# nyx-space/nyx

Hardware: AMD Instinct MI355X
Metric: propagated trajectories/sec (10k-ensemble, 1-day RK89) (higher is better)
Workload: dtype f64

## Files before the change

### nyx_amd/csrc/pk_integrator_ool.h

```cpp
#ifndef INTEG_OOL
#define INTEG_OOL ((NYX_EMIT & (NYX_EMIT_PLAIN16 | NYX_EMIT_PLAIN16_P2 | NYX_EMIT_PLAIN16_FAN)) ? 1 : 0)
#endif
#if INTEG_OOL
#define IX_HOT 1
#define IX_SPEC_NOW 2
#define IX_COOP 4
#define IX_PROF 8
#define IX_SHARED 16
#define IXR_ANSWER 0x10000
#define IXR_FALLBACK 0x20000
DEVFN char *lds_from_u32(uint32_t a) { return (char *)(__attribute__((address_space(3))) char *)(uintptr_t)a; }
DEVFN LdsPtr ix_rows(const double *arr, int lane) {
    uint32_t a = (uint32_t)(uintptr_t)(LdsCPtr)arr + (uint32_t)lane * 8u;
    asm volatile("" : "+v"(a));
    return (LdsPtr)(uintptr_t)a;
}
DEVFN void ix_stamp(LdsFlagPtr ctl, int k) {
    const int64_t t = (int64_t)__builtin_readcyclecounter();
    ctl[8 + 2 * k] = (int)(uint32_t)t; ctl[9 + 2 * k] = (int)(uint32_t)(t >> 32);
}
#define IX_PROLOGUE                                                                                                        \
    CfgPtr cfg = (CfgPtr)uniform_u64(cfg_u);                                                                               \
    const LdsMap L = carve_lds(lds_from_u32(__builtin_amdgcn_readfirstlane(lds_v)), 0, false, cfg->rec_in_lds ? cfg->rec_doubles : 0, cfg->ed_reuse, false); \
    double *const kbuf = L.kbuf;                                                                                           \
    double *const tabl = L.tabl;                                                                                           \
    constexpr int KB_STR = DEV_LANES;                                                                                      \
    const int kb_li = lane;                                                                                                \
    const int i = __builtin_amdgcn_readfirstlane(i_v);                                                                     \
    const int flags = __builtin_amdgcn_readfirstlane(flags_v);                                                             \
    const int stages = cfg->stages;

static __device__ __attribute__((noinline)) int integ_front(uint32_t lds_v, uint64_t cfg_u, int i_v, int flags_v, int lane, double h,
                                                           double v3, double v4, double v5, double p0, double p1, double p2,
                                                           uint64_t cbox_u, uint64_t posted_u, uint32_t seq_nx_v, int keep_k0) {
    IX_PROLOGUE
    const bool has_grav = cfg->has_grav != 0;
    const bool need_almanac = has_grav || cfg->has_drag != 0 || cfg->has_tides != 0 || cfg->n_slots > 0;
    const bool spec = cfg->spec != 0;
    int st = NYX_HIP_OK;
    double vel[3] = {v3, v4, v5};
    if (flags & IX_HOT) {
        double *const ysb = (i & 1) ? L.ys2 : L.ys;
        if (i == 0) {
#pragma unroll
            for (int e = 0; e < 3; ++e) vel[e] = CS_Y(3 + e);
        } else {
            const double a_last = A_ROW(i, i - 1);
            const double w[3] = {v3, v4, v5};
#pragma unroll
            for (int e = 0; e < 3; ++e) {
                const double wi = w[e] + a_last * KB(i - 1, 3 + e);
                vel[e] = CS_Y(3 + e) + h * wi;
            }
        }
#pragma unroll
        for (int e = 0; e < 3; ++e) ysb[(3 + e) * DEV_LANES + lane] = vel[e];
        if (cfg->has_drag) {
            __builtin_amdgcn_fence(__ATOMIC_RELEASE, "workgroup");
            if (lane == 0) LCTL[4] = i + 1;
        }
        if (need_almanac && !(i == 0 && keep_k0)) {
            const int n_alm = cfg->n_alm;
            for (int a = 0; a < n_alm; ++a) {
                const int es = L.edst[(2 * a + (i & 1)) * DEV_LANES + lane];
                if (es) st = es;
            }
        }
// ... 15 lines not shown
        }
        double *const ysn = ((i + 1) & 1) ? L.ys2 : L.ys;
        double *const inbn = ((i + 1) & 1) ? L.inb2 : L.inb;
#pragma unroll
        for (int e = 0; e < 3; ++e) ysn[e * DEV_LANES + lane] = nx_pos[e];
        if (has_grav) {
            if (need_almanac) {
                int spin = 0;
                while (LCTL[2] != i + 1 && ++spin < 4000000) __builtin_amdgcn_s_sleep(4);
                if (spin >= 4000000) st = NYX_HIP_ERR_NAN;
                __builtin_amdgcn_fence(__ATOMIC_ACQUIRE, "workgroup");
            }
            const double *const edn = L.ed + ((i + 1) & 1) * ED_FIELDS * DEV_LANES;
            double m_nx[9];
#pragma unroll
            for (int q = 0; q < 9; ++q) m_nx[q] = edn[q * DEV_LANES + lane];
            const double rb0 = m_nx[0] * nx_pos[0] + m_nx[1] * nx_pos[1] + m_nx[2] * nx_pos[2];
            const double rb1 = m_nx[3] * nx_pos[0] + m_nx[4] * nx_pos[1] + m_nx[5] * nx_pos[2];
            const double rb2 = m_nx[6] * nx_pos[0] + m_nx[7] * nx_pos[1] + m_nx[8] * nx_pos[2];
            const double r_ = norm3(rb0, rb1, rb2);
            const double inv_r = 1.0 / r_;
            const double nx_s = rb0 * inv_r, nx_t = rb1 * inv_r, nx_u = rb2 * inv_r;
            const double rho = cfg->g_re * inv_r;
            const double nx_kfac = (cfg->g_mu * inv_r) * cfg->g_inv_re;
            inbn[0 * DEV_LANES + lane] = rho * nx_s;
            inbn[1 * DEV_LANES + lane] = rho * nx_t;
            inbn[2 * DEV_LANES + lane] = rho * nx_u;
            inbn[3 * DEV_LANES + lane] = rho;
            inbn[4 * DEV_LANES + lane] = r_ * cfg->g_inv_re;
            double *const sx = ((i + 1) & 1) ? L.ixs : L.part;
            sx[0 * DEV_LANES + lane] = nx_s; sx[1 * DEV_LANES + lane] = nx_t; sx[2 * DEV_LANES + lane] = nx_u; sx[3 * DEV_LANES + lane] = nx_kfac;
        }
        if (lane == 0) L.ctl[1] = (flags & IX_COOP) ? 1 : 0;
        if ((flags & IX_COOP) && has_grav) {
            CoopBox *const cbox = (CoopBox *)uniform_u64(cbox_u);
            uint32_t *const posted = (uint32_t *)uniform_u64(posted_u);
            const uint32_t seq_nx = (uint32_t)__builtin_amdgcn_readfirstlane((int)seq_nx_v);
            if (flags & IX_PROF) ix_stamp(LCTL, 1);
            coop_post_inl(cbox, posted, lane, seq_nx, (LdsCPtr)inbn, COOP_PARTS_HERE);
            if (flags & IX_PROF) ix_stamp(LCTL, 2);
        }
    }
    return st;
}

struct IxBack {
    double px, py, pz, pw;
    int ret;
};
#define IXR_NEED_FB 0x40000
DEVFN void ix_assemble(CfgPtr cfg, const LdsMap &L, int i, int lane, double (&acc)[3], double px, double py, double pz, double pw,
                       const double (&m_cur)[9], double s_, double t_, double u_, double kfac, int skip_k) {
    const LdsPtr pertc = ix_rows((i & 1) ? L.pert2 : L.pert, lane);
    const LdsPtr ysb = ix_rows((i & 1) ? L.ys2 : L.ys, lane);
    const LdsPtr kb = ix_rows(L.kbuf + i * 6 * DEV_LANES, lane);
    if (cfg->has_grav) {
        px *= kfac; py *= kfac; pz *= kfac; pw *= kfac;
        const double al0 = px + pw * s_, al1 = py + pw * t_, al2 = pz + pw * u_;
        acc[0] += m_cur[0] * al0 + m_cur[3] * al1 + m_cur[6] * al2;
        acc[1] += m_cur[1] * al0 + m_cur[4] * al1 + m_cur[7] * al2;
        acc[2] += m_cur[2] * al0 + m_cur[5] * al1 + m_cur[8] * al2;
    }
    if (cfg->has_srp) {
        acc[0] += pertc[3 * DEV_LANES]; acc[1] += pertc[4 * DEV_LANES]; acc[2] += pertc[5 * DEV_LANES];
    }
    if (cfg->has_drag) {
        acc[0] += pertc[6 * DEV_LANES]; acc[1] += pertc[7 * DEV_LANES]; acc[2] += pertc[8 * DEV_LANES];
    }
    if (!skip_k) {
        kb[0 * DEV_LANES] = ysb[3 * DEV_LANES]; kb[1 * DEV_LANES] = ysb[4 * DEV_LANES]; kb[2 * DEV_LANES] = ysb[5 * DEV_LANES];
        kb[3 * DEV_LANES] = acc[0]; kb[4 * DEV_LANES] = acc[1]; kb[5 * DEV_LANES] = acc[2];
    }
}
static __device__ __attribute__((noinline)) IxBack integ_back(uint32_t lds_v, uint64_t cfg_u, int i_v, int flags_v, int lane, double a0, double a1,
                                                             double a2, double px, double py, double pz, double pw, uint32_t seq_cur_v, int fold_val_v,
// ... 210 lines not shown
```

### nyx_amd/csrc/pk_state_lds.h

```cpp

#define NIN 5
#define DBG_SKIP_SERIAL 0x100
#define DBG_SKIP_HARMONICS 0x200
#define KB(stage, comp) kbuf[((stage)*6 + (comp)) * KB_STR + kb_li]

#define CS_FIELDS 21
static __device__ __attribute__((noinline)) bool event_step(const nyx_hip_event_t *ev, double mu, int64_t epoch_ns, double *prev, int32_t *count,
                                                            double y0, double y1, double y2, double y3, double y4, double y5) {
    const double y[6] = {y0, y1, y2, y3, y4, y5};
    const double y_next = ev_eval(*ev, mu, epoch_ns, y);
    int n = *count;
    if (ev_crossing(ev->scalar, *prev, y_next)) n += 1;
    *prev = y_next;
    *count = n;
    return n >= ev->trigger;
}

struct ColdState {
    int64_t epoch, stop, step_size, prev_step, det_step, n_acc, n_rej, n_evals;
    double y[9];
    double h, det_error;
    int det_attempts, attempts, status;
    bool done, fresh, is_final, fixed, prev_kind, backprop, massless;
};
// ... 108 lines not shown
               2 * ED_FIELDS * DEV_LANES + 2 * DEV_LANES + CS_FIELDS * DEV_LANES + (size_t)(quad ? DEV_MAX_WAVES * QSLOT : DEV_MAX_WAVES * 4 * DEV_LANES) + DEV_MAX_ALM * DEV_LANES +
               DEV_LANES + 8 + (size_t)rec_doubles;
    d += quad ? (size_t)(10 + 15 + 6 + QPRE_ROWS + 6 + 10 + 15) * DEV_LANES : (stm ? (size_t)(20 + 27 + 12) * DEV_LANES : (size_t)(NIN + 9 + 6 + NIN + 9 + 4) * DEV_LANES);
    (void)n_waves;
    if (reuse_fields > 0) d += (size_t)reuse_fields * DEV_LANES + 2 * DEV_LANES + DEV_LANES / 2;
    return d * sizeof(double) + 64;
}

DEVFN void begin_attempt_fn(const LdsMap &L, int lane, ColdState &c) {
    if (!c.done && c.fresh) {
        if ((!c.backprop && c.epoch + c.step_size > c.stop) || (c.backprop && c.epoch + c.step_size <= c.stop)) {
            if (c.stop == c.epoch) {
                c.done = true;
            } else {
                c.prev_step = c.step_size;
                c.prev_kind = c.fixed;
                c.step_size = c.stop - c.epoch;
                c.fixed = true;
                c.is_final = true;
            }
        }
        c.attempts = 1;
        c.h = ns_to_seconds(c.step_size);
        c.fresh = false;
    }
    if (!c.done && c.massless) { c.status = NYX_HIP_ERR_MASSLESS; c.done = true; }
    L.step[lane] = __longlong_as_double(c.epoch);
    L.step[DEV_LANES + lane] = c.h;
    if (!__any(!c.done)) {
        if (lane == 0) L.ctl[0] = 1;
    }
}

#define PROF_T0() const int64_t pt0_ = prof_on ? (int64_t)__builtin_readcyclecounter() : 0
#define PROF_ADD(slot) if (prof_on) prof_acc[slot] += (int64_t)__builtin_readcyclecounter() - pt0_
#define A_ROW(i, j) tabl[(i)*DEV_MAX_STAGES + (j)]
#define B_COEF(i) tabl[DEV_MAX_STAGES * DEV_MAX_STAGES + (i)]
#define BD_COEF(i) tabl[DEV_MAX_STAGES * DEV_MAX_STAGES + DEV_MAX_STAGES + (i)]
#define C_COEF(i) tabl[DEV_MAX_STAGES * DEV_MAX_STAGES + 2 * DEV_MAX_STAGES + (i)]

static __device__ __attribute__((noinline)) bool stm_update_textbook(double *phi, double h, const double *hist, int64_t stride, int64_t gid, double *kb,
                                                                  const double *tabl, int stages_v, int lane) {
    const int stages = __builtin_amdgcn_readfirstlane(stages_v);
    bool nan = false;
    for (int col = 0; col < 9; ++col) {
        double p[6];
#pragma unroll
        for (int e = 0; e < 6; ++e) p[e] = phi[e + 9 * col];
        const double gam = phi[6 + 9 * col];
        for (int i = 0; i < stages; ++i) {
            double wi[6] = {0.0, 0.0, 0.0, 0.0, 0.0, 0.0};
            for (int j = 0; j < i; ++j) {
                const double a_ij = A_ROW(i, j);
#pragma unroll
                for (int e = 0; e < 6; ++e) wi[e] += a_ij * kb[(j * 6 + e) * DEV_LANES + lane];
            }
            double ps[6];
#pragma unroll
            for (int e = 0; e < 6; ++e) ps[e] = p[e] + h * wi[e];
            double g[12];
#pragma unroll
            for (int q = 0; q < 12; ++q) g[q] = hist[(int64_t)(i * 12 + q) * stride + gid];
#pragma unroll
            for (int a = 0; a < 3; ++a) {
                double s = g[3 * a + 0] * ps[0];
                s += g[3 * a + 1] * ps[1];
// ... 25 lines not shown
```

### nyx_amd/csrc/propagate_kernel.hip

```cpp

#include <hip/hip_runtime.h>

#include <mutex>

#include "../../include/nyx_hip.h"
#include "devcfg.h"
#include "hifitime_dev.h"
#include "event_dev.h"
#include "predict_args.h"

#ifndef NYX_EMIT
#define NYX_EMIT 1
#endif
#define NYX_EMIT_PLAIN16 1
#define NYX_EMIT_PLAIN8 2
#define NYX_EMIT_STM 4
#define NYX_EMIT_STMQ16 8
#define NYX_EMIT_STMQ8 16
#define NYX_EMIT_PLAIN16_P2 32
#define NYX_EMIT_PLAIN8N 64
#define NYX_EMIT_PLAIN16_FAN 128
#ifndef NYX_PROF
#define NYX_PROF 0
#endif
#define NYX_HOST_TU ((NYX_EMIT & NYX_EMIT_PLAIN16) && !NYX_PROF)
#ifdef NYX_COOP_TWO_PARTS
#define COOP_PARTS_HERE 2
#else
#define COOP_PARTS_HERE 1
#endif

#define CAS __attribute__((address_space(4)))
typedef const CAS DevCfg *CfgPtr;
typedef const CAS HarmEntry *HarmPtr;
typedef const CAS ColHdr *ColPtr;

#define DEVFN static __device__ __forceinline__
typedef const __attribute__((address_space(3))) double *LdsCPtr;
typedef volatile __attribute__((address_space(3))) int *LdsFlagPtr;
#define LCTL ((LdsFlagPtr)L.ctl)

DEVFN double norm3(double x, double y, double z) { return sqrt(x * x + y * y + z * z); }
DEVFN double cube(double x) { return x * (x * x); }
DEVFN double clamp02(double x) { return x < 0.0 ? 0.0 : (x > 2.0 ? 2.0 : x); }

#include "pk_epoch_data.h"
#include "pk_force_models.h"
#include "pk_harmonics.h"
#include "pk_cooperative.h"
#include "pk_error_stm.h"
#include "pk_state_lds.h"
#include "pk_integrator_ool.h"
#include "pk_segment_update.h"
template <bool INTEG, bool ALMANAC, bool PERT, bool STM, bool QUAD = false, bool PIPE = false>
DEVFN void role_loop(const DevBatch &bt, CfgPtr cfg, const DevCfg *cfg_g, HarmPtr htab, ColPtr cols,
                     const double *__restrict__ records, const LdsMap &L, const int lane, const int wave, const int nw) {
    double *const kbuf = L.kbuf;
    double *const tabl = L.tabl;
    const int stages = cfg->stages;
    asm volatile("s_nop 13\n\ts_nop %0" ::"n"((INTEG ? 1 : 0) | (ALMANAC ? 2 : 0) | (PERT ? 4 : 0) | (PIPE ? 8 : 0)) : "memory");
#ifdef NYX_ASSUME_SMALL
    const bool has_grav = false, has_drag = false, has_tides = false, has_grav2 = false;
// ... 62 lines not shown
        }
        if (bt.traj_cap > 0 && wr) {
            bt.t_epoch[gid] = c.epoch;
#pragma unroll
            for (int e = 0; e < 6; ++e) bt.t_state[e][gid] = c.y[e];
            bt.t_len[gid] = (duration == 0 || c.done) ? 1 : 1;
        }
        if (STM && valid && bt.o_stm != bt.stm) {
            for (int q = ql; q < 81; q += (QUAD ? 4 : 1)) bt.o_stm[gid * 81 + q] = bt.stm[gid * 81 + q];
        }
    }
    if (PERT) {
        p_cr = clamp02(bt.cr ? bt.cr[idx] : 0.0);
        p_area = bt.asrp ? bt.asrp[idx] : 0.0;
        p_cd = bt.cd ? bt.cd[idx] : 0.0;
        p_darea = bt.adrag ? bt.adrag[idx] : 0.0;
        p_mass = (bt.mdry ? bt.mdry[idx] : 0.0) + (bt.mprop ? bt.mprop[idx] : 0.0) + (bt.mextra ? bt.mextra[idx] : 0.0);
    }
    __syncthreads();
    CoopBox *const cbox = bt.coop_box + blockIdx.x;
    const int coop_widx = bt.coop_sets > 0 ? ((int)blockIdx.x % bt.coop_sets) * COOP_SET + (int)blockIdx.x / bt.coop_sets : 0;
#define coop_two (COOP_PARTS_HERE == 2)
#ifdef NYX_COOP_FAN
#define COOP_FB_PARTS ((bt.coop_parts & 0xf) << 8)
#else
#define COOP_FB_PARTS (coop_two ? 0x100 : 0)
#endif
    bool coop_on = !STM && LCTL[1] != 0;
    const bool coop_started = coop_on;
    uint32_t coop_seq = 0;
    bool coop_drop = false;
    static_assert(!PIPE || ((!STM || QUAD) && !(INTEG && (ALMANAC || PERT))), "the pipelined stage loop needs the integrator in a wave of its own");
    constexpr bool pipe = PIPE;
    RotBase rot_base;
    rot_base.ep = INT64_MIN;
#pragma unroll
    for (int q = 0; q < 3; ++q) { rot_base.sn[q] = 0.0; rot_base.cs[q] = 1.0; }
    const int reuse_nf = (!STM && ALMANAC && !INTEG && need_almanac && cfg->n_alm == 1) ? cfg->ed_reuse : 0;
    if (reuse_nf > 0) { L.ed0_ep[lane] = INT64_MIN; L.spec_ep[lane] = INT64_MIN; }
    const bool spec = pipe && !STM && cfg->spec != 0;
    const bool offl = PIPE && !STM && !INTEG_OOL && cfg->offload != 0;
    const bool qoff = STM && QUAD && cfg->qpre_off != 0;
#if INTEG_OOL
    constexpr bool ool = PIPE && !STM;
    const uint32_t lds_base = (uint32_t)(uintptr_t)(LdsPtr)L.kbuf;
#define IX_STAMP(k) (int64_t)(((uint64_t)(uint32_t)LCTL[9 + 2 * (k)] << 32) | (uint64_t)(uint32_t)LCTL[8 + 2 * (k)])
#else
    constexpr bool ool = false;
#endif
    bool spec_now = false;
    bool keep_k0 = false;
    int att = 0;
    double nx_pos[3] = {0.0, 0.0, 0.0}, nx_s = 0.0, nx_t = 0.0, nx_u = 0.0, nx_kfac = 0.0;
    double m_cur[9], m_nx[9];
#pragma unroll
    for (int q = 0; q < 9; ++q) { m_cur[q] = 0.0; m_nx[q] = 0.0; }
    uint32_t seq_cur = 0, seq_nx = 0;
    unsigned long long dbg_answers = 0, dbg_fallbacks = 0, dbg_fb_seq = 0;
    int64_t pl_tc = 0, pl_chain = 0, pl_wait = 0, pl_n = 0, pl_post = 0;
#if NYX_SEG_PROF
    int64_t sg[16] = {0, 0, 0, 0, 0, 0, 0, 0, 0, 0, 0, 0, 0, 0, 0, 0}, sg_t = 0;
#define SEG(k) if (INTEG && prof_on) { const int64_t n_ = (int64_t)__builtin_readcyclecounter(); sg[k] += n_ - sg_t; sg_t = n_; }
    int64_t sb[8] = {0, 0, 0, 0, 0, 0, 0, 0}, sb_t = 0;
#define SBD(k) if (INTEG && STM && prof_on) { const int64_t n_ = (int64_t)__builtin_readcyclecounter(); if (sb_t) sb[k] += n_ - sb_t; sb_t = n_; }
#else
#define SEG(k)
// ... 47 lines not shown
                cold_store(L.cs, lane, c);
                h = c.h;
            }
            __syncthreads();
            SBD(4)
        }
        if (LCTL[0]) break;
        }

        if (!spec_now && ALMANAC && need_almanac) {
            const int64_t ep = __double_as_longlong(L.step[lane]);
            bool compute = true;
            if (reuse_nf > 0) {
                const bool hit_spec = ep == (int64_t)L.spec_ep[lane];
                const bool hit_prev = ep == (int64_t)L.ed0_ep[lane];
                compute = __any(!(hit_spec || hit_prev)) != 0;
                if (!compute && !hit_spec) {
                    for (int f = 0; f < reuse_nf; ++f) L.ed[f * DEV_LANES + lane] = L.ed0[f * DEV_LANES + lane];
                    my_edst[lane] = L.ed0st[lane];
                }
            }
            if (compute) {
                int st = rec_in_lds ? epoch_data(cfg, (const double *)L.rec, ep, L.ed, lane, amask, nullptr, 0, &rot_base)
                                    : epoch_data(cfg, records, ep, L.ed, lane, amask, nullptr, 0, &rot_base);
                my_edst[lane] = st;
            }
            if (reuse_nf > 0) {
                for (int f = 0; f < reuse_nf; ++f) L.ed0[f * DEV_LANES + lane] = L.ed[f * DEV_LANES + lane];
                L.ed0st[lane] = my_edst[lane];
                L.ed0_ep[lane] = ep;
            }
        }
        if (!spec_now) {
        if (INTEG && lane == 0) { L.ctl[2] = 0; L.ctl[3] = 0; L.ctl[4] = 0; L.ctl[6] = 0; }
        __syncthreads();
        SBD(5)
        }
        const int fold_base = spec ? att * stages : 0;
        bool leave = false;

        int st_att = NYX_HIP_OK;
        double wpre[6] = {0.0, 0.0, 0.0, 0.0, 0.0, 0.0};
        double pre_wr[3] = {0.0, 0.0, 0.0};
        for (int i = 0; i < stages; ++i) {
            double *const edc = L.ed + (i & 1) * ED_FIELDS * DEV_LANES;
            double s_ = 0.0, t_ = 0.0, u_ = 0.0, kfac = 0.0;
            double ys[6];
            PROF_T0();
            SEG(0)
            if (INTEG) {
                double *const ysb = (pipe && (i & 1)) ? L.ys2 : L.ys;
                double *const inbb = (pipe && (i & 1)) ? L.inb2 : L.inb;
                if (ool && pipe && (i > 0 || spec_now)) {
                    seq_cur = seq_nx; shared_cur = shared_nx;
                } else
                if (!ool && pipe && (i > 0 || spec_now)) {
                    if (i == 0) {
#pragma unroll
                        for (int e = 0; e < 6; ++e) ys[e] = CS_Y(e);
#pragma unroll
                        for (int e = 3; e < 6; ++e) ysb[e * DEV_LANES + lane] = ys[e];
                    } else {
                    const double a_last = A_ROW(i, i - 1);
                    if (!STM) {
#pragma unroll
                        for (int e = 0; e < 3; ++e) ys[e] = ysb[e * DEV_LANES + lane];
                    } else {
#pragma unroll
                    for (int e = 0; e < 3; ++e) ys[e] = nx_pos[e];
                    }
#pragma unroll
                    for (int e = 3; e < 6; ++e) {
                        const double wi = wpre[e] + a_last * KB(i - 1, e);
                        ys[e] = CS_Y(e) + h * wi;
                        ysb[e * DEV_LANES + lane] = ys[e];
                    }
// ... 70 lines not shown
                        const D3 sD = d3div(x0, rD), tD = d3div(x1, rD), uD = d3div(x2, rD);
                        const D3 rhoD = d3div(d3c(cfg->g_re), rD);
                        const D3 kD = d3div(d3div(d3c(cfg->g_mu), rD), d3c(cfg->g_re));
                        const D3 invD = rD * cfg->g_inv_re;
                        (void)kD;
                        const D3 pub[5] = {rhoD * sD, rhoD * tD, rhoD * uD, rhoD, invD};
#pragma unroll
                        for (int q = 0; q < 5; ++q) {
                            L.inbD[(4 * q + 0) * DEV_LANES + lane] = pub[q].v; L.inbD[(4 * q + 1) * DEV_LANES + lane] = pub[q].x;
                            L.inbD[(4 * q + 2) * DEV_LANES + lane] = pub[q].y; L.inbD[(4 * q + 3) * DEV_LANES + lane] = pub[q].z;
                        }
                    }
                }
                if (pipe) {
                    shared_cur = coop_on;
                    if (lane == 0) L.ctl[1] = coop_on ? 1 : 0;
                }
                if (ool) {
                    L.part[0 * DEV_LANES + lane] = s_; L.part[1 * DEV_LANES + lane] = t_; L.part[2 * DEV_LANES + lane] = u_; L.part[3 * DEV_LANES + lane] = kfac;
                }
                }
            }
            PROF_ADD(0);
            SEG(1)
            if (!pipe || (i == 0 && !spec_now)) {
                PROF_T0();
                __syncthreads();
                PROF_ADD(6);
            }
#if NYX_SEG_PROF
            if (i == 0) { SBD(6) }
            if (i == 1) sb_t = 0;
#endif
            const int64_t ptw_ = prof_on ? (int64_t)__builtin_readcyclecounter() : 0;

            if (INTEG && !STM && coop_on && has_grav && (!pipe || (i == 0 && !spec_now))) {
                seq_cur = ++coop_seq;
                if (coop_two) coop_post2(cbox, bt.coop_posted + coop_widx, lane, seq_cur, (LdsCPtr)L.inb); else coop_post(cbox, bt.coop_posted + coop_widx, lane, seq_cur, (LdsCPtr)L.inb);
            }
            const bool last_stage = i + 1 == stages;
            if (ALMANAC && need_almanac && (!last_stage || reuse_nf > 0 || spec)) {
                if (spec_now && i == 0) {
                    int spin = 0;
                    while (LCTL[5] != att && ++spin < 4000000) __builtin_amdgcn_s_sleep(4);
                    __builtin_amdgcn_fence(__ATOMIC_ACQUIRE, "workgroup");
                }
                const double c_next = last_stage ? 1.0 : C_COEF(i + 1);
                const int64_t ep = __double_as_longlong(L.step[lane]) + seconds_to_ns(c_next * L.step[DEV_LANES + lane]);
                double *edn = L.ed + ((i + 1) & 1) * ED_FIELDS * DEV_LANES;
                if (last_stage && reuse_nf > 0) L.spec_ep[lane] = ep;
                int st = NYX_HIP_OK;
                if (!dbg_skip_serial || i == 0)
                {
                    const LdsFlagPtr fl = (pipe && (!last_stage || spec) && (amask & DEV_ROLE_DCM)) ? LCTL + 2 : nullptr;
                    const LdsFlagPtr gt = ool ? LCTL + 3 : nullptr;
                    st = rec_in_lds ? epoch_data(cfg, (const double *)L.rec, ep, edn, lane, amask, fl, i + 1, &rot_base, gt, fold_base + i)
                                    : epoch_data(cfg, records, ep, edn, lane, amask, fl, i + 1, &rot_base, gt, fold_base + i);
                }
                my_edst[((i + 1) & 1) * DEV_LANES + lane] = st;
                if (pipe && (!last_stage || spec) && (amask & DEV_ROLE_DCM)) {
                    asm volatile("s_waitcnt lgkmcnt(0)" ::: "memory");
                    if (lane == 0) LCTL[2] = i + 1;
                }
            }
            if (PIPE && !STM && ALMANAC && offl) {
                if (amask & DEV_ROLE_TWOBODY) {
                    const double *const ysp = (i & 1) ? L.ys2 : L.ys;
                    const double r0 = ysp[0 * DEV_LANES + lane], r1 = ysp[1 * DEV_LANES + lane], r2 = ysp[2 * DEV_LANES + lane];
                    const double rmag = norm3(r0, r1, r2);
                    const double f = -cfg->mu_central / cube(rmag);
                    double *const tb = L.part + (12 + 3 * (i & 1)) * DEV_LANES;
                    tb[0 * DEV_LANES + lane] = f * r0; tb[1 * DEV_LANES + lane] = f * r1; tb[2 * DEV_LANES + lane] = f * r2;
                }
                if ((amask & DEV_ROLE_SUMS) && i >= 2 && i + 2 < stages) {
                    double q6[6] = {0.0, 0.0, 0.0, 0.0, 0.0, 0.0};
#pragma unroll 4
                    for (int j = 0; j <= i - 2; ++j) {
                        const double a_nj = A_ROW(i + 2, j);
#pragma unroll
                        for (int e = 0; e < 6; ++e) q6[e] += a_nj * KB(j, e);
                    }
                    double *const qb = L.part + (i & 1) * 6 * DEV_LANES;
#pragma unroll
                    for (int e = 0; e < 6; ++e) qb[e * DEV_LANES + lane] = q6[e];
                }
            }
            if (ALMANAC && STM && QUAD && qoff && (amask & DEV_ROLE_QPRE)) {
                bool expired = false;
                if (i > 0) {
                    int spin = 0;
                    while (LCTL[6] < i && ++spin < 4000000) __builtin_amdgcn_s_sleep(2);
                    expired = spin >= 4000000;
                    __builtin_amdgcn_fence(__ATOMIC_ACQUIRE, "workgroup");
                }
                if (expired) my_edst[((i + 1) & 1) * DEV_LANES + lane] = NYX_HIP_ERR_NAN;
                const double *const ysq = (pipe && (i & 1)) ? L.ys2 : L.ys;
                if (!expired) quad_pre(cfg, edc, ysq[0 * DEV_LANES + lane], ysq[1 * DEV_LANES + lane], ysq[2 * DEV_LANES + lane], ql, lane, L.qpre, has_grav);
            }
            if (PERT && (has_pm || has_srp || has_drag || has_tides || has_grav2)) {
                double *const ysp = (pipe && (i & 1)) ? L.ys2 : L.ys;
                double *const pertp = (pipe && (i & 1)) ? L.pert2 : L.pert;
                double r[3] = {ysp[0 * DEV_LANES + lane], ysp[1 * DEV_LANES + lane], ysp[2 * DEV_LANES + lane]};
                const bool do_pm = (pmask & DEV_PERT_PM) != 0, do_srp = (pmask & DEV_PERT_SRP) != 0;
                if (!STM) {
                    double a3[3] = {0.0, 0.0, 0.0}, f3[3] = {0.0, 0.0, 0.0};
                    if (has_pm && do_pm && !dbg_skip_serial) point_masses_accel(cfg, edc, lane, r, a3);
                    if (has_srp && do_srp && !dbg_skip_serial) {
                        srp_force(cfg, edc, lane, r, p_cr, p_area, f3);
                        f3[0] = f3[0] / p_mass; f3[1] = f3[1] / p_mass; f3[2] = f3[2] / p_mass;
                    }
                    if (do_pm) {
#pragma unroll
                        for (int e = 0; e < 3; ++e) pertp[e * DEV_LANES + lane] = a3[e];
                    }
                    if (do_srp) {
#pragma unroll
                        for (int e = 0; e < 3; ++e) pertp[(3 + e) * DEV_LANES + lane] = f3[e];
                    }
                }
                if (has_drag && do_srp) {
                    if (pipe && (i > 0 || spec_now)) {
                        int spin = 0;
                        while (LCTL[4] != i + 1 && ++spin < 4000000) __builtin_amdgcn_s_sleep(4);
                        __builtin_amdgcn_fence(__ATOMIC_ACQUIRE, "workgroup");
                    }
                    const double vv[3] = {ysp[3 * DEV_LANES + lane], ysp[4 * DEV_LANES + lane], ysp[5 * DEV_LANES + lane]};
                    const int64_t ep = __double_as_longlong(L.step[lane]) + seconds_to_ns(C_COEF(i) * L.step[DEV_LANES + lane]);
                    double d3f[3];
                    drag_force(cfg, rec_in_lds ? (const double *)L.rec : records, edc, lane, ns_to_seconds(ep), r, vv, p_cd, p_darea, d3f);
#pragma unroll
                    for (int e = 0; e < 3; ++e) pertp[(6 + e) * DEV_LANES + lane] = d3f[e] / p_mass;
                }
// ... 68 lines not shown
                    nx_s = rb0 * inv_r; nx_t = rb1 * inv_r; nx_u = rb2 * inv_r;
                    const double rho = cfg->g_re * inv_r;
                    nx_kfac = (cfg->g_mu * inv_r) * cfg->g_inv_re;
                    inbn[0 * DEV_LANES + lane] = rho * nx_s;
                    inbn[1 * DEV_LANES + lane] = rho * nx_t;
                    inbn[2 * DEV_LANES + lane] = rho * nx_u;
                    inbn[3 * DEV_LANES + lane] = rho;
                    inbn[4 * DEV_LANES + lane] = r_ * cfg->g_inv_re;
                    if (STM && QUAD) publish_d1_inputs(cfg, rb0, rb1, rb2, ql, inbn, lane);
                    if (!STM) {
                        L.part[0 * DEV_LANES + lane] = nx_s; L.part[1 * DEV_LANES + lane] = nx_t; L.part[2 * DEV_LANES + lane] = nx_u; L.part[3 * DEV_LANES + lane] = nx_kfac;
                    }
                    }
                    SEG(4)
                    shared_nx = coop_on;
                    if (lane == 0) L.ctl[1] = coop_on ? 1 : 0;
                    if (coop_on) {
                        seq_nx = ++coop_seq;
                        const int64_t p0_ = prof_on ? (int64_t)__builtin_readcyclecounter() : 0;
                        if (coop_two) coop_post2(cbox, bt.coop_posted + coop_widx, lane, seq_nx, (LdsCPtr)inbn); else coop_post(cbox, bt.coop_posted + coop_widx, lane, seq_nx, (LdsCPtr)inbn);
                        if (prof_on && pl_tc != 0) { const int64_t now_ = (int64_t)__builtin_readcyclecounter(); pl_chain += p0_ - pl_tc; pl_post += now_ - p0_; ++pl_n; pl_tc = 0; }
                    }
                }
            };
#if INTEG_OOL
            if (INTEG && fastp && ool) {
                const bool hot = i > 0 || spec_now;
                const bool pub = i + 1 < stages || spec;
                uint32_t sq = 0;
                if (pub && coop_on) sq = ++coop_seq;
                const int64_t pf0_ = prof_on ? (int64_t)__builtin_readcyclecounter() : 0;
                const int st1 = integ_front(lds_base, (uint64_t)cfg, i, (hot ? IX_HOT : 0) | (spec_now ? IX_SPEC_NOW : 0) | (coop_on ? IX_COOP : 0) | (prof_on ? IX_PROF : 0),
                                            lane, h, hot ? wpre[3] : ys[3], hot ? wpre[4] : ys[4], hot ? wpre[5] : ys[5], pre_wr[0], pre_wr[1], pre_wr[2],
                                            (uint64_t)cbox, (uint64_t)(bt.coop_posted + coop_widx), sq, keep_k0 ? 1 : 0);
                if (prof_on) prof_acc[0] += (int64_t)__builtin_readcyclecounter() - pf0_;
                SEG(5)
                if (st1) st_att = st1;
                if (pub) {
                    shared_nx = coop_on;
                    if (coop_on) {
                        seq_nx = sq;
                        if (prof_on && pl_tc != 0) { const int64_t p0_ = IX_STAMP(1), now_ = IX_STAMP(2); pl_chain += p0_ - pl_tc; pl_post += now_ - p0_; ++pl_n; pl_tc = 0; }
                    }
                }
                {
                    const double *const ysb = (i & 1) ? L.ys2 : L.ys;
#pragma unroll
                    for (int e = 0; e < 6; ++e) ys[e] = ysb[e * DEV_LANES + lane];
                    if (hot && i == 0) {
#pragma unroll
                        for (int e = 0; e < 3; ++e) ys[e] = CS_Y(e);
                    }
                }
                {
                    const double rmag = norm3(ys[0], ys[1], ys[2]);
                    const double f = -cfg->mu_central / cube(rmag);
                    acc[0] = f * ys[0]; acc[1] = f * ys[1]; acc[2] = f * ys[2];
                }
#pragma unroll
                for (int e = 0; e < 6; ++e) wpre[e] = 0.0;
                if (i + 1 < stages) {
#pragma unroll
                    for (int j = 0; j < DEV_MAX_STAGES - 2; ++j) {
                        if (j < i) {
                            const double a_nj = A_ROW(i + 1, j);
#pragma unroll
                            for (int e = 3; e < 6; ++e) wpre[e] += a_nj * KB(j, e);
// ... 114 lines not shown
            }
            if (INTEG && STM && QUAD && !qoff) quad_pre(cfg, edc, ys[0], ys[1], ys[2], ql, lane, L.qpre, has_grav);
            SEG(6)
            if (prof_on) prof_acc[1] += (int64_t)__builtin_readcyclecounter() - ptw_;
            const int64_t pth_ = prof_on ? (int64_t)__builtin_readcyclecounter() : 0;
            double px = 0.0, py = 0.0, pz = 0.0, pw = 0.0;
            double coop_x = 0.0, coop_y = 0.0, coop_z = 0.0, coop_w = 0.0;
            if (has_grav && dbg_skip_harm && !INTEG) {
                double *pp = L.part + wave * 4 * DEV_LANES;
                pp[0 * DEV_LANES + lane] = 0.0; pp[1 * DEV_LANES + lane] = 0.0;
                pp[2 * DEV_LANES + lane] = 0.0; pp[3 * DEV_LANES + lane] = 0.0;
            }
            if (STM && QUAD) {
                if (has_grav && cfg->sched[DEV_SCHED_SOLO].n_ranges[wave] > 0)
                    harmonics_partial_d1((uint64_t)cfg, (uint64_t)htab, (uint64_t)cols, wave, (LdsCPtr)((pipe && (i & 1)) ? L.inb2 : L.inbD),
                                         (LdsPtr)(L.partD + wave * QSLOT), lane, LCTL + 3, pipe ? i : 0);
            } else if (STM && has_grav)
                harmonics_partial_dual((uint64_t)cfg, (uint64_t)htab, (uint64_t)cols, wave, L.inbD, L.partD + wave * 16 * DEV_LANES, lane);
            if (!STM && has_grav && !dbg_skip_harm) {
                const int sched = LCTL[1] ? DEV_SCHED_PRIMARY : DEV_SCHED_SOLO;
                const double *const inbw = (pipe && (i & 1)) ? L.inb2 : L.inb;
                Partial4 pr = {0.0, 0.0, 0.0, 0.0};
#ifdef NYX_COOP_FAN
                if (!(pipe && INTEG) && (sched == DEV_SCHED_PRIMARY ? rows_primary : rows_solo)) {
#else
                if (!(pipe && INTEG)) {
#endif
                    const double v0 = inbw[0 * DEV_LANES + lane], v1 = inbw[1 * DEV_LANES + lane], v2 = inbw[2 * DEV_LANES + lane],
                                 v3 = inbw[3 * DEV_LANES + lane], v4 = inbw[4 * DEV_LANES + lane];
                    pr = (cfg->harm_feed & 1) ? harmonics_stream((uint64_t)cfg, (uint64_t)cols, wave, sched, v0, v1, v2, v3, v4)
                                        : harmonics_partial((uint64_t)cfg, (uint64_t)htab, (uint64_t)cols, wave, sched, v0, v1, v2, v3, v4);
                }
                px = pr.x; py = pr.y; pz = pr.z; pw = pr.w;
                if (!INTEG) {
                    if (pipe && (i > 0 || spec_now)) {
                        int spin = 0;
                        while (LCTL[3] < fold_base + i && ++spin < 4000000) __builtin_amdgcn_s_sleep(1);
                    }
                    double *pp = L.part + wave * 4 * DEV_LANES;
                    pp[0 * DEV_LANES + lane] = px; pp[1 * DEV_LANES + lane] = py;
                    pp[2 * DEV_LANES + lane] = pz; pp[3 * DEV_LANES + lane] = pw;
                }
            }
#define COOP_COLLECT()                                                                                                                          \
            if (INTEG && !STM && has_grav && (pipe ? shared_cur : coop_on)) {                                                                     \
                const CoopAnswer ans = !coop_on ? CoopAnswer{0.0, 0.0, 0.0, 0.0, 0} : (coop_two ? coop_wait2(cbox, bt.coop_out2 + blockIdx.x, lane, seq_cur) : coop_wait(cbox, lane, seq_cur)); \
                if (ans.ok) {                                                                                                                     \
                    coop_x = ans.x; coop_y = ans.y; coop_z = ans.z; coop_w = ans.w;                                                               \
                    ++dbg_answers;                                                                                                                \
                } else {                                                                                                                          \
                    if (coop_on) { ++dbg_fallbacks; dbg_fb_seq = seq_cur; }   \
                    const Partial4 fb = coop_fallback((uint64_t)cfg, (uint64_t)htab, (uint64_t)cols, (pipe && (i & 1)) ? L.inb2 : L.inb, lane | COOP_FB_PARTS); \
                    coop_x = fb.x; coop_y = fb.y; coop_z = fb.z; coop_w = fb.w;                                                                   \
                    coop_on = false;                                                                                                              \
                    coop_drop = !pipe;                                     \
                    if (lane == 0) coop_store(bt.coop_finished + coop_widx, 1u);                                                                  \
                }                                                                                                                                 \
            }
            if (!pipe && !ool) {
                const int64_t w0_ = prof_on ? (int64_t)__builtin_readcyclecounter() : 0;
                COOP_COLLECT()
                if (prof_on && INTEG) { pl_tc = (int64_t)__builtin_readcyclecounter(); pl_wait += pl_tc - w0_; }
            }
            if (prof_on) prof_acc[2] += (int64_t)__builtin_readcyclecounter() - pth_;
            {
                PROF_T0();
                __syncthreads();
                PROF_ADD(6);
            }
            SEG(7)
            if (spec_now && i == 0 && LCTL[0]) {
                leave = true;
                break;
            }
            const int64_t ptc_ = prof_on ? (int64_t)__builtin_readcyclecounter() : 0;

#if INTEG_OOL
            if (INTEG && ool) {
                const int skip_k = (spec_now && i == 0 && keep_k0) ? 1 : 0;
                const Partial4 f4 = fold_partials((LdsCPtr)L.part, lane, 0.0, 0.0, 0.0, 0.0);
                const IxBack rb_ = integ_back(lds_base, (uint64_t)cfg, i, (shared_cur ? IX_SHARED : 0) | (coop_on ? IX_COOP : 0) | (prof_on ? IX_PROF : 0), lane,
                                              acc[0], acc[1], acc[2], f4.x, f4.y, f4.z, f4.w, seq_cur, fold_base + i + 1, (uint64_t)cbox,
                                              (uint64_t)(bt.coop_out2 + blockIdx.x), skip_k);
                if (rb_.ret & 0xffff) st_att = rb_.ret & 0xffff;
                if (rb_.ret & IXR_ANSWER) ++dbg_answers;
                if (rb_.ret & IXR_NEED_FB) {
                    if (coop_on) { ++dbg_fallbacks; dbg_fb_seq = seq_cur; }
                    const Partial4 fb = coop_fallback((uint64_t)cfg, (uint64_t)htab, (uint64_t)cols, (i & 1) ? L.inb2 : L.inb, lane | COOP_FB_PARTS);
                    integ_back_slow(lds_base, (uint64_t)cfg, (uint64_t)records, i, lane, acc[0], acc[1], acc[2], rb_.px, rb_.py, rb_.pz, rb_.pw, fb.x, fb.y, fb.z, fb.w, skip_k);
                    coop_on = false;
                    if (lane == 0) coop_store(bt.coop_finished + coop_widx, 1u);
                }
                if (prof_on && shared_cur) { pl_tc = IX_STAMP(0); pl_wait += pl_tc - IX_STAMP(3); }
            } else
#endif
            if (INTEG) {
                const double *const pertc = (pipe && (i & 1)) ? L.pert2 : L.pert;
                if (offl) {
// ... 101 lines not shown
                            tmp[3 * a + 2] = m[0 + a] * al[0].z + m[3 + a] * al[1].z + m[6 + a] * al[2].z;
                        }
#pragma unroll
                        for (int a = 0; a < 3; ++a)
#pragma unroll
                            for (int b = 0; b < 3; ++b)
                                G[3 * a + b] += tmp[3 * a + 0] * m[0 + b] + tmp[3 * a + 1] * m[3 + b] + tmp[3 * a + 2] * m[6 + b];
                    }
                    if (has_srp) {
#pragma unroll
                        for (int q = 0; q < 3; ++q) { acc[q] += L.pertD[(12 + q) * DEV_LANES + lane]; cv[q] = L.pertD[(24 + q) * DEV_LANES + lane]; }
#pragma unroll
                        for (int q = 0; q < 9; ++q) G[q] += L.pertD[(15 + q) * DEV_LANES + lane];
                    }
                    const double b_i = B_COEF(i);
#pragma unroll
                    for (int q = 0; q < 9; ++q) L.sacc[q * DEV_LANES + lane] += b_i * G[q];
#pragma unroll
                    for (int q = 0; q < 3; ++q) L.sacc[(9 + q) * DEV_LANES + lane] += b_i * cv[q];
                    if (bt.stm_hist != nullptr && valid) {
#pragma unroll
                        for (int q = 0; q < 9; ++q) bt.stm_hist[(int64_t)(i * 12 + q) * bt.stm_hist_stride + gid] = G[q];
#pragma unroll
                        for (int q = 0; q < 3; ++q) bt.stm_hist[(int64_t)(i * 12 + 9 + q) * bt.stm_hist_stride + gid] = cv[q];
                    }
                }
                if (!(STM && QUAD) && !(spec_now && i == 0 && keep_k0)) {
                    KB(i, 0) = ys[3]; KB(i, 1) = ys[4]; KB(i, 2) = ys[5];
                    KB(i, 3) = acc[0]; KB(i, 4) = acc[1]; KB(i, 5) = acc[2];
                }
            }
            SEG(10)
            if (prof_on) prof_acc[3] += (int64_t)__builtin_readcyclecounter() - ptc_;
        }
        if (leave) break;

        const int64_t pts_ = prof_on ? (int64_t)__builtin_readcyclecounter() : 0;
#if NYX_SEG_PROF
        if (INTEG && STM && prof_on) sb_t = (int64_t)__builtin_readcyclecounter();
#endif
        keep_k0 = false;
#if INTEG_OOL && STEP_OOL
        if (INTEG && ool && !bt.ev_on) {
            const IxStep sr = integ_step(lds_base, (uint64_t)cfg, lane, h, st_att, att, spec ? IXS_CHAIN : 0);
            keep_k0 = (sr.ret & IXS_KEEP_K0) != 0;
            if (spec) h_next = sr.h_next;
            if ((sr.ret & IXS_ACCEPT) && bt.traj_cap > 0 && wr) {
                const int64_t acc_n = __double_as_longlong(L.cs[5 * DEV_LANES + lane]);
                if (acc_n < bt.traj_cap) {
                    const int64_t at = acc_n * bt.n + gid;
                    bt.t_epoch[at] = __double_as_longlong(L.cs[0 * DEV_LANES + lane]);
#pragma unroll
                    for (int e = 0; e < 6; ++e) bt.t_state[e][at] = CS_Y(e);
                }
                bt.t_len[gid] = (int32_t)(acc_n + 1);
            }
        } else
#endif
        if (INTEG) {
            ColdState c;
            cold_load(L.cs, lane, c);
            double *const y = c.y;
            if (!c.done) c.n_evals += stages;
            SEG(12)
            double next[9], err[9];
#pragma unroll
// ... 363 lines not shown
```

Measured before the change: 16980.

## Replace per-stage workgroup barrier with LDS arrive/publish flags in pipelined loop

In the pipelined, non-STM configurations, the per-stage __syncthreads is replaced by LDS counters. Harmonics waves write their partials and atomically bump an arrival counter. The integrator wave spins until all waves have arrived and publishes a stage word from integ_front, which the other waves wait on before reading the state. This is meant to remove full-workgroup barrier stalls and let waves proceed as soon as their own dependencies are met. In exchange it adds spin-wait sleeps, s_nop padding and release/acquire fences, and it risks ordering bugs or timeouts reported as NaN errors.

```diff
diff --git a/nyx_amd/csrc/pk_integrator_ool.h b/nyx_amd/csrc/pk_integrator_ool.h
--- a/nyx_amd/csrc/pk_integrator_ool.h
+++ b/nyx_amd/csrc/pk_integrator_ool.h
@@ -19,6 +19,13 @@
     const int64_t t = (int64_t)__builtin_readcyclecounter();
     ctl[8 + 2 * k] = (int)(uint32_t)t; ctl[9 + 2 * k] = (int)(uint32_t)(t >> 32);
 }
+#if STAGE_FLAGS
+#define IX_PUB_PARAM , int pub_v
+#define IX_PUB_ARG(v) , (v)
+#else
+#define IX_PUB_PARAM
+#define IX_PUB_ARG(v)
+#endif
 #define IX_PROLOGUE                                                                                                        \
     CfgPtr cfg = (CfgPtr)uniform_u64(cfg_u);                                                                               \
     const LdsMap L = carve_lds(lds_from_u32(__builtin_amdgcn_readfirstlane(lds_v)), 0, false, cfg->rec_in_lds ? cfg->rec_doubles : 0, cfg->ed_reuse, false); \
@@ -32,7 +39,7 @@
 
 static __device__ __attribute__((noinline)) int integ_front(uint32_t lds_v, uint64_t cfg_u, int i_v, int flags_v, int lane, double h,
                                                            double v3, double v4, double v5, double p0, double p1, double p2,
-                                                           uint64_t cbox_u, uint64_t posted_u, uint32_t seq_nx_v, int keep_k0) {
+                                                           uint64_t cbox_u, uint64_t posted_u, uint32_t seq_nx_v, int keep_k0 IX_PUB_PARAM) {
     IX_PROLOGUE
     const bool has_grav = cfg->has_grav != 0;
     const bool need_almanac = has_grav || cfg->has_drag != 0 || cfg->has_tides != 0 || cfg->n_slots > 0;
@@ -114,6 +121,10 @@
             sx[0 * DEV_LANES + lane] = nx_s; sx[1 * DEV_LANES + lane] = nx_t; sx[2 * DEV_LANES + lane] = nx_u; sx[3 * DEV_LANES + lane] = nx_kfac;
         }
         if (lane == 0) L.ctl[1] = (flags & IX_COOP) ? 1 : 0;
+#if STAGE_FLAGS
+        __builtin_amdgcn_fence(__ATOMIC_RELEASE, "workgroup");
+        if (lane == 0) LCTL[SF_PUBLISHED] = __builtin_amdgcn_readfirstlane(pub_v);
+#endif
         if ((flags & IX_COOP) && has_grav) {
             CoopBox *const cbox = (CoopBox *)uniform_u64(cbox_u);
             uint32_t *const posted = (uint32_t *)uniform_u64(posted_u);
@@ -123,6 +134,11 @@
             if (flags & IX_PROF) ix_stamp(LCTL, 2);
         }
     }
+#if STAGE_FLAGS
+    else {
+        if (lane == 0) LCTL[SF_PUBLISHED] = __builtin_amdgcn_readfirstlane(pub_v);
+    }
+#endif
     return st;
 }
 
diff --git a/nyx_amd/csrc/pk_state_lds.h b/nyx_amd/csrc/pk_state_lds.h
--- a/nyx_amd/csrc/pk_state_lds.h
+++ b/nyx_amd/csrc/pk_state_lds.h
@@ -164,6 +164,22 @@
     }
 }
 
+#if STAGE_FLAGS
+#define SF_ARRIVED 6
+#define SF_PUBLISHED 7
+DEVFN void sf_arrive(volatile __attribute__((address_space(3))) int *ctl, int lane) {
+    __builtin_amdgcn_fence(__ATOMIC_RELEASE, "workgroup");
+    if (lane == 0) asm volatile("ds_add_u32 %0, %1" ::"v"((uint32_t)(uintptr_t)(ctl + SF_ARRIVED)), "v"(1) : "memory");
+}
+DEVFN bool sf_wait(volatile __attribute__((address_space(3))) int *word, unsigned want) {
+    int spin = 0;
+#pragma nounroll
+    while ((int)((unsigned)*word - want) < 0 && ++spin < 4000000) __builtin_amdgcn_s_sleep(1);
+    __builtin_amdgcn_fence(__ATOMIC_ACQUIRE, "workgroup");
+    return spin < 4000000;
+}
+#endif
+
 #define PROF_T0() const int64_t pt0_ = prof_on ? (int64_t)__builtin_readcyclecounter() : 0
 #define PROF_ADD(slot) if (prof_on) prof_acc[slot] += (int64_t)__builtin_readcyclecounter() - pt0_
 #define A_ROW(i, j) tabl[(i)*DEV_MAX_STAGES + (j)]
diff --git a/nyx_amd/csrc/propagate_kernel.hip b/nyx_amd/csrc/propagate_kernel.hip
--- a/nyx_amd/csrc/propagate_kernel.hip
+++ b/nyx_amd/csrc/propagate_kernel.hip
@@ -28,6 +28,10 @@
 #define COOP_PARTS_HERE 2
 #else
 #define COOP_PARTS_HERE 1
+#endif
+
+#ifndef STAGE_FLAGS
+#define STAGE_FLAGS ((NYX_EMIT & (NYX_EMIT_PLAIN16 | NYX_EMIT_PLAIN16_P2)) ? 1 : 0)
 #endif
 
 #define CAS __attribute__((address_space(4)))
@@ -156,6 +160,8 @@
     bool coop_drop = false;
     static_assert(!PIPE || ((!STM || QUAD) && !(INTEG && (ALMANAC || PERT))), "the pipelined stage loop needs the integrator in a wave of its own");
     constexpr bool pipe = PIPE;
+    constexpr bool sflags = STAGE_FLAGS && PIPE && !STM;
+    static_assert(!sflags || INTEG_OOL, "the published word is raised in integ_front");
     RotBase rot_base;
     rot_base.ep = INT64_MIN;
 #pragma unroll
@@ -269,16 +275,20 @@
             }
         }
         if (!spec_now) {
-        if (INTEG && lane == 0) { L.ctl[2] = 0; L.ctl[3] = 0; L.ctl[4] = 0; L.ctl[6] = 0; }
+        if (INTEG && lane == 0) { L.ctl[2] = 0; L.ctl[3] = 0; L.ctl[4] = 0; if (!sflags) L.ctl[6] = 0; }
         __syncthreads();
         SBD(5)
         }
         const int fold_base = spec ? att * stages : 0;
+        const unsigned ev_base = (unsigned)att * (unsigned)stages;
         bool leave = false;
 
         int st_att = NYX_HIP_OK;
         double wpre[6] = {0.0, 0.0, 0.0, 0.0, 0.0, 0.0};
         double pre_wr[3] = {0.0, 0.0, 0.0};
+#if STAGE_FLAGS
+#pragma nounroll
+#endif
         for (int i = 0; i < stages; ++i) {
             double *const edc = L.ed + (i & 1) * ED_FIELDS * DEV_LANES;
             double s_ = 0.0, t_ = 0.0, u_ = 0.0, kfac = 0.0;
@@ -415,6 +425,7 @@
             if (i == 0) { SBD(6) }
             if (i == 1) sb_t = 0;
 #endif
+            if (sflags) asm volatile("s_nop 12" ::: "memory");
             const int64_t ptw_ = prof_on ? (int64_t)__builtin_readcyclecounter() : 0;
 
             if (INTEG && !STM && coop_on && has_grav && (!pipe || (i == 0 && !spec_now))) {
@@ -423,6 +434,9 @@
             }
             const bool last_stage = i + 1 == stages;
             if (ALMANAC && need_almanac && (!last_stage || reuse_nf > 0 || spec)) {
+#if STAGE_FLAGS
+                if (sflags && !(amask & DEV_ROLE_DCM) && (i > 0 || spec_now)) (void)sf_wait(LCTL + 3, (unsigned)(fold_base + i));
+#endif
                 if (spec_now && i == 0) {
                     int spin = 0;
                     while (LCTL[5] != att && ++spin < 4000000) __builtin_amdgcn_s_sleep(4);
@@ -481,6 +495,9 @@
                 if (!expired) quad_pre(cfg, edc, ysq[0 * DEV_LANES + lane], ysq[1 * DEV_LANES + lane], ysq[2 * DEV_LANES + lane], ql, lane, L.qpre, has_grav);
             }
             if (PERT && (has_pm || has_srp || has_drag || has_tides || has_grav2)) {
+#if STAGE_FLAGS
+                if (sflags && (i > 0 || spec_now)) (void)sf_wait(LCTL + 3, (unsigned)(fold_base + i));
+#endif
                 double *const ysp = (pipe && (i & 1)) ? L.ys2 : L.ys;
                 double *const pertp = (pipe && (i & 1)) ? L.pert2 : L.pert;
                 double r[3] = {ysp[0 * DEV_LANES + lane], ysp[1 * DEV_LANES + lane], ysp[2 * DEV_LANES + lane]};
@@ -615,7 +632,7 @@
                 const int64_t pf0_ = prof_on ? (int64_t)__builtin_readcyclecounter() : 0;
                 const int st1 = integ_front(lds_base, (uint64_t)cfg, i, (hot ? IX_HOT : 0) | (spec_now ? IX_SPEC_NOW : 0) | (coop_on ? IX_COOP : 0) | (prof_on ? IX_PROF : 0),
                                             lane, h, hot ? wpre[3] : ys[3], hot ? wpre[4] : ys[4], hot ? wpre[5] : ys[5], pre_wr[0], pre_wr[1], pre_wr[2],
-                                            (uint64_t)cbox, (uint64_t)(bt.coop_posted + coop_widx), sq, keep_k0 ? 1 : 0);
+                                            (uint64_t)cbox, (uint64_t)(bt.coop_posted + coop_widx), sq, keep_k0 ? 1 : 0 IX_PUB_ARG((int)(ev_base + (unsigned)i + 1u)));
                 if (prof_on) prof_acc[0] += (int64_t)__builtin_readcyclecounter() - pf0_;
                 SEG(5)
                 if (st1) st_att = st1;
@@ -796,7 +813,11 @@
                                         : harmonics_partial((uint64_t)cfg, (uint64_t)htab, (uint64_t)cols, wave, sched, v0, v1, v2, v3, v4);
                 }
                 px = pr.x; py = pr.y; pz = pr.z; pw = pr.w;
+#if STAGE_FLAGS
+                if (!INTEG && !sflags) {
+#else
                 if (!INTEG) {
+#endif
                     if (pipe && (i > 0 || spec_now)) {
                         int spin = 0;
                         while (LCTL[3] < fold_base + i && ++spin < 4000000) __builtin_amdgcn_s_sleep(1);
@@ -827,7 +848,30 @@
                 if (prof_on && INTEG) { pl_tc = (int64_t)__builtin_readcyclecounter(); pl_wait += pl_tc - w0_; }
             }
             if (prof_on) prof_acc[2] += (int64_t)__builtin_readcyclecounter() - pth_;
-            {
+            if (sflags) {
+#if STAGE_FLAGS
+                const unsigned ev = ev_base + (unsigned)i;
+                PROF_T0();
+                if (INTEG) {
+                    if (!sf_wait(LCTL + SF_ARRIVED, (unsigned)(nw - 1) * (ev + 1u))) st_att = NYX_HIP_ERR_NAN;
+                } else {
+#pragma nounroll
+                    for (int spin = 0; spin < 4000000; ++spin) {
+                        const int folded = LCTL[3] - (fold_base + i), published = (int)((unsigned)LCTL[SF_PUBLISHED] - (ev + 1u));
+                        if ((folded | published) >= 0) break;
+                        __builtin_amdgcn_s_sleep(1);
+                    }
+                    __builtin_amdgcn_fence(__ATOMIC_ACQUIRE, "workgroup");
+                }
+                PROF_ADD(6);
+                if (!INTEG) {
+                    double *pp = L.part + wave * 4 * DEV_LANES;
+                    pp[0 * DEV_LANES + lane] = px; pp[1 * DEV_LANES + lane] = py;
+                    pp[2 * DEV_LANES + lane] = pz; pp[3 * DEV_LANES + lane] = pw;
+                    sf_arrive(LCTL, lane);
+                }
+#endif
+            } else {
                 PROF_T0();
                 __syncthreads();
                 PROF_ADD(6);
@@ -995,6 +1039,7 @@
             }
             SEG(10)
             if (prof_on) prof_acc[3] += (int64_t)__builtin_readcyclecounter() - ptc_;
+            if (sflags) asm volatile("s_nop 11" ::: "memory");
         }
         if (leave) break;
 
```

New measurement: 16680. 0.983x the previous value.
